# Changfei-Fu/RUMI-SLAM

Measured on AMD Instinct MI355X. Metric: frames/sec ORB extract+match, higher is better.
Workload: dtype u8; 1 GPU; ORB extract (640x480, 8-level pyramid, 1000 features/frame) + brute-force 256-bit Hamming match of consecutive frames (BASELINE.json configs[1]+[2]); scaling=n/a (one GPU), exchange=none

## Files before the change

rumi_slam_amd/csrc/orb_device.h:

```cpp
#pragma once
#include <hip/hip_runtime.h>

#include <cstdint>

#include "orb_geom.h"
#include "rumi_orb.h"

namespace rumi {

struct DevLevel {
    int w, h, pitch;
    long long off;
    int nCols, nRows, wCell, hCell;
    int cellBase, nCells;
    int maxBX, maxBY;
    int nfeat;
    float scale;
    float patchSize;
    int candCap;
    int coefX, coefXT, coefY, xmax;
    int xmaxFast;
    int rowTab;
};

struct DevParams {
    int nlevels, totalCells, maxCellCand, totalCand;
    int iniTh, minTh;
    long long arenaStride;
    int umax[16];
    DevLevel lv[kMaxLevels];
};

struct ImgSrc {
    const uint8_t *l0;
    long long l0FrameStride;
    int l0Pitch;
    uint8_t *pyr;
    uint8_t *blur;
};

struct RowTap { int32_t r0, r1; uint32_t bh0, bh1; };
struct PyrTile { int16_t x0[kMaxLevels], x1[kMaxLevels], y0[kMaxLevels], y1[kMaxLevels]; };
void launch_pyramid_tiles(const DevParams *dP, ImgSrc src, const int16_t *coef, const RowTap *rowTab, const PyrTile *tiles, int ntiles, int bufBytes,
                          int tabEntries, int nframes, hipStream_t st, int32_t *clearWord = nullptr, bool copyL0 = false);
void launch_resize(const DevParams *dP, const DevParams &hP, ImgSrc src, const int16_t *coef, const RowTap *rowTab, int level, int nframes,
                   hipStream_t st, int32_t *clearWord = nullptr);
void launch_fast(const DevParams *dP, const DevParams &hP, ImgSrc src, uint32_t *cellBuf, int32_t *cellCnt, int nframes,
                 hipStream_t st);
bool fast_blur_fusable(const DevParams &hP);
bool launch_fast_blur(const DevParams *dP, const DevParams &hP, ImgSrc src, uint32_t *cellBuf, int32_t *cellCnt, int nframes, int variant, hipStream_t st);
void launch_compact(const DevParams *dP, const DevParams &hP, const uint32_t *cellBuf, const int32_t *cellCnt,
                    uint32_t *cand, int32_t *levelStart, int32_t *errFlag, int nframes, hipStream_t st);
void launch_blur(const DevParams *dP, const DevParams &hP, ImgSrc src, int nframes, int variant, hipStream_t st);
void launch_orient_desc(const DevParams *dP, ImgSrc src, const uint32_t *selPacked, const uint32_t *selMeta,
                        const int32_t *selCount, int selCap, int maxSel, RumiKeyPoint *kpOut, long long kpStride, uint8_t *descOut,
                        long long descStride, int outCap, int nframes, hipStream_t st);

void launch_assemble_orient_desc(const DevParams *dP, ImgSrc src, const uint32_t *selLevel, const int32_t *selLevelCnt, int selLevelCap, int lap0, int lap1,
                                 int32_t *counts, long long countsStride, int32_t *errFlag, int32_t *errMirror, uint32_t *selPacked, uint32_t *selMeta,
                                 int32_t *selCount, int selCap, int maxSel, RumiKeyPoint *kpOut,
                                 long long kpStride, uint8_t *descOut, long long descStride, int outCap, int nframes, hipStream_t st);
void launch_octree(const DevParams *dP, const DevParams &hP, const uint32_t *cand, const int32_t *levelStart,
                   uint16_t *owner, uint32_t *selLevel, int32_t *selLevelCnt, int selLevelCap, int32_t *errFlag,
                   int nframes, size_t ldsBytes, hipStream_t st);
void launch_assemble(const DevParams *dP, const uint32_t *selLevel, const int32_t *selLevelCnt, int selLevelCap, int lap0,
                     int lap1, uint32_t *selPacked, uint32_t *selMeta, int32_t *selCount, int selCap, int32_t *counts, long long countsStride,
                     int32_t *errFlag, int nframes, hipStream_t st, int32_t *errMirror = nullptr);
size_t octree_lds_for(const DevParams &hP);

}
```

rumi_slam_amd/csrc/orb_host.hip:

```cpp
#include <hip/hip_runtime.h>

#include <cstdlib>

#include <algorithm>
#include <atomic>
#include <cstdio>
#include <cstring>
#include <functional>
#include <string>
#include <thread>
#include <vector>

#include "orb_device.h"
#include "orb_octree.h"
#include "rumi_common.h"

using namespace rumi;

namespace rumi {
thread_local std::string g_lastError;
void set_error(const char *fmt, const char *a, const char *b, int line) {
    char buf[512];
    snprintf(buf, sizeof buf, fmt, a, b, line);
    g_lastError = buf;
// ... 38 lines not shown
    RowTap *dRowTab = nullptr; int capRowTab = 0;
    PyrTile *dPyrTiles[2] = {nullptr, nullptr}; int nPyrTiles[2] = {0, 0}, pyrBuf[2] = {0, 0}, pyrTab[2] = {0, 0};
    uint8_t *dIn = nullptr;
    uint8_t *dL0 = nullptr;
    uint8_t *hIn = nullptr, *hOut1 = nullptr, *dOut1 = nullptr;
    size_t out1Bytes = 0;
    uint8_t *dhOut1 = nullptr;
    int32_t *dhErr = nullptr;
    bool zeroCopyOut = false;
    uint8_t *dhIn = nullptr;
    bool hostImagePending = false;
    uint8_t *dPyr = nullptr, *dBlur = nullptr;
    uint32_t *dCellBuf = nullptr;
    int32_t *dCellCnt = nullptr;
    uint32_t *dCand = nullptr;
    int32_t *dLevelStart = nullptr;
    uint32_t *dSelPacked = nullptr, *dSelMeta = nullptr;
    int32_t *dSelCount = nullptr;
    RumiKeyPoint *dKp = nullptr;
    uint8_t *dDesc = nullptr;
    int32_t *dCounts = nullptr;
    uint16_t *dOwner = nullptr;
    uint32_t *dSelLevel = nullptr;
    int32_t *dSelLevelCnt = nullptr;
    int32_t *dErr = nullptr;
    uint8_t *dHostIn = nullptr; size_t dHostInBytes = 0;
    static constexpr int kFeedSlots = 4, kFeedFrames = 64;
    uint8_t *hFeed[kFeedSlots] = {nullptr}; size_t hFeedBytes = 0;
    hipEvent_t evFeed[kFeedSlots] = {nullptr};
    hipStream_t copyStream = nullptr, copyStream2 = nullptr;
    std::function<int(int, hipStream_t)> feed;
    bool pending = false;
    hipStream_t pendingStream = nullptr;
    int selLevelCap = 0;
    size_t octLds = 0;
    int32_t *hErr = nullptr;
    std::vector<uint32_t> tapCand, tapSelPacked, tapSelMeta;
    std::vector<int32_t> tapLevelStart, tapSelCount;
    bool tapValid = false;
    ImgSrc lastSrc{};
    int lastFrames = 0, lastChunkBase = 0, lastChunkFrames = 0, lastChunkSlot = 0;
    RumiKeyPoint *lastKp = nullptr;
    long long lastKpStride = 0;
    int32_t *lastCounts = nullptr;
    int lastOutCap = 0;
    bool profiling = false;
    float stageMs[8] = {0};
    struct Mirror { uint8_t *host; const uint8_t *dev; long long row; } mirror[3] = {{nullptr, nullptr, 0}, {nullptr, nullptr, 0}, {nullptr, nullptr, 0}};
    hipEvent_t ev[8] = {nullptr};
    hipStream_t sideStream = nullptr;
    static constexpr int kMaxParts = 8;
    hipStream_t partStream[kMaxParts - 1] = {nullptr}, partSide[kMaxParts - 1] = {nullptr};
    bool residentQueue = false;
    int residentSlots = 4;
    int scratchFrames = 0, arenaFrames = 0;
    int rot = 0;
    hipEvent_t userReady = nullptr;
    bool lastResident = false;
    hipStream_t part0Stream = nullptr, part0Side = nullptr;
    hipEvent_t evPart0Join = nullptr, evSide0Fork = nullptr, evSide0Join = nullptr;
    hipEvent_t evPartFork = nullptr, evPartJoin[kMaxParts - 1] = {nullptr}, evSideFork[kMaxParts - 1] = {nullptr}, evSideJoin[kMaxParts - 1] = {nullptr};
    hipEvent_t evFork = nullptr, evJoin = nullptr, evB0 = nullptr, evB1 = nullptr;
};

static int set_geometry(RumiOrb *h, int w, int hgt) {
    if (h->gw == w && h->gh == hgt) return RUMI_OK;
    std::vector<LevelGeom> g;
    long long arena; int cells, cand, cellCand;
    if (!make_geometry(h->tab, w, hgt, g, &arena, &cells, &cand, &cellCand)) {
        g_lastError = "image too small for the FAST cell grid at some pyramid level, or cell larger than the LDS tile";
        return RUMI_E_INVALID;
    }
    if (arena > h->capArena || cells > h->capCells || cand > h->capCand || cellCand > h->capCellCand) {
        g_lastError = "image larger than the handle's max_width x max_height arenas";
        return RUMI_E_CAPACITY;
    }
    DevParams &P = h->hP;
    std::memset(&P, 0, sizeof P);
    P.nlevels = h->tab.nlevels; P.totalCells = cells; P.maxCellCand = h->capCellCand; P.totalCand = h->capCand;
    P.iniTh = std::min(std::max(h->cfg.ini_th_fast, 0), 255);
    P.minTh = std::min(std::max(h->cfg.min_th_fast, 0), 255);
    P.arenaStride = h->capArena;
    for (int i = 0; i < 16; i++) P.umax[i] = h->tab.umax[i];
    std::vector<int16_t> coef;
    std::vector<RowTap> rowTab;
    for (int l = 0; l < P.nlevels; l++) {
        DevLevel &D = P.lv[l];
        const LevelGeom &G = g[l];
        D.w = G.w; D.h = G.h; D.pitch = G.pitch; D.off = G.off;
        D.nCols = G.nCols; D.nRows = G.nRows; D.wCell = G.wCell; D.hCell = G.hCell;
        D.cellBase = G.cellBase; D.nCells = G.nCells; D.maxBX = G.maxBX; D.maxBY = G.maxBY;
        D.nfeat = G.nfeat; D.scale = G.scale;
        D.patchSize = (float)(int)(kPatchSize * G.scale);
        D.candCap = std::min(G.candCap, 65535);
        D.coefX = D.coefXT = D.coefY = 0; D.xmax = D.xmaxFast = G.w; D.rowTab = 0;
        if (l > 0) {
            std::vector<int16_t> ofs, taps;
            int dmax;
            make_resize_axis(g[l - 1].w, G.w, true, ofs, taps, &dmax);
            D.coefX = (int)coef.size(); D.xmax = dmax;
            D.xmaxFast = dmax == G.w ? G.w + 3 : dmax;
            for (int k = 0; k < 4; k++) { ofs.push_back(ofs[G.w - 1]); taps.push_back(taps[2 * G.w - 2]); taps.push_back(taps[2 * G.w - 1]); }
            coef.insert(coef.end(), ofs.begin(), ofs.end());
            D.coefXT = (int)coef.size();
            coef.insert(coef.end(), taps.begin(), taps.end());
            make_resize_axis(g[l - 1].h, G.h, false, ofs, taps, &dmax);
            D.coefY = (int)coef.size();
            coef.insert(coef.end(), ofs.begin(), ofs.end());
            coef.insert(coef.end(), taps.begin(), taps.end());
            D.rowTab = (int)rowTab.size();
            const int sh = g[l - 1].h;
            for (int oy = 0; oy < G.h; oy++) {
                const int sy = ofs[oy];
                const int sy0 = sy >= 0 ? (sy < sh ? sy : sh - 1) : 0, sy1r = sy + 1, sy1 = sy1r >= 0 ? (sy1r < sh ? sy1r : sh - 1) : 0;
                rowTab.push_back(RowTap{sy0, sy1, (uint32_t)taps[oy * 2] << 16, (uint32_t)taps[oy * 2 + 1] << 16});
            }
        }
    }
    if ((int)coef.size() > h->capCoef) { g_lastError = "resize table capacity"; return RUMI_E_CAPACITY; }
    HIP_TRY(hipMemcpy(h->dP, &P, sizeof P, hipMemcpyHostToDevice));
    if ((int)rowTab.size() > h->capRowTab) { g_lastError = "resize row table capacity"; return RUMI_E_CAPACITY; }
    if (!coef.empty()) HIP_TRY(hipMemcpy(h->dCoef, coef.data(), coef.size() * sizeof(int16_t), hipMemcpyHostToDevice));
    if (!rowTab.empty()) HIP_TRY(hipMemcpy(h->dRowTab, rowTab.data(), rowTab.size() * sizeof(RowTap), hipMemcpyHostToDevice));
    auto build_tiles = [&](int kPyrTX, int kPyrTY, int set) -> int {
        h->nPyrTiles[set] = 0; h->pyrBuf[set] = 0;
        if (P.nlevels < 2) return RUMI_OK;
        const int top = P.nlevels - 1;
        const int ntx = (P.lv[top].w + kPyrTX - 1) / kPyrTX, nty = (P.lv[top].h + kPyrTY - 1) / kPyrTY;
        std::vector<PyrTile> tiles((size_t)ntx * nty);
        int bufMax = 0, tabMax = 0, dimMax = 0, winRows = 0, winCols = 0;
        auto up4 = [](int x) { return (x + 3) & ~3; };
        for (int ty = 0; ty < nty; ty++)
            for (int tx = 0; tx < ntx; tx++) {
                PyrTile &T = tiles[(size_t)ty * ntx + tx];
                std::memset(&T, 0, sizeof T);
                int x0 = 0, x1 = 0, y0 = 0, y1 = 0, tab = 0;
                for (int l = top; l >= 0; l--) {
                    const DevLevel &D = P.lv[l];
                    int ox0 = (int)((long long)D.w * tx / ntx), ox1 = (int)((long long)D.w * (tx + 1) / ntx);
                    int oy0 = (int)((long long)D.h * ty / nty), oy1 = (int)((long long)D.h * (ty + 1) / nty);
                    if (l < top) {
                        const DevLevel &U = P.lv[l + 1];
                        const int16_t *xofs = coef.data() + U.coefX;
                        const int nx0 = xofs[x0], nx1 = std::min(D.w, (int)xofs[x1 - 1] + 2);
                        const int ny0 = rowTab[(size_t)U.rowTab + y0].r0, ny1 = rowTab[(size_t)U.rowTab + y1 - 1].r1 + 1;
                        if (l == 0) { ox0 = nx0; ox1 = nx1; oy0 = ny0; oy1 = ny1; }
                        else { ox0 = std::min(ox0, nx0); ox1 = std::max(ox1, nx1); oy0 = std::min(oy0, ny0); oy1 = std::max(oy1, ny1); }
                    }
                    if (l > 0) { x0 = ox0 & ~3; x1 = up4(ox1); } else { x0 = ox0 & ~3; x1 = ox1; }
                    y0 = oy0; y1 = oy1;
                    T.x0[l] = (int16_t)x0; T.x1[l] = (int16_t)x1; T.y0[l] = (int16_t)y0; T.y1[l] = (int16_t)y1;
                    bufMax = std::max(bufMax, up4(x1 - x0) * (y1 - y0));
                    if (l > 0) tab += (x1 - x0) + (y1 - y0);
                    if (l > 0) dimMax = std::max(dimMax, std::max(x1 - x0, y1 - y0));
                    if (l == 0) { winRows = std::max(winRows, y1 - y0); winCols = std::max(winCols, x1 - x0); }
                }
                tabMax = std::max(tabMax, tab);
            }
        bufMax = (bufMax + 15) & ~15;
        if (2 * bufMax + 8 * tabMax <= 60 * 1024 && tiles.size() <= 4096 && P.nlevels <= 8 && dimMax <= 256 && winRows <= 80 && winCols <= 256) {
            if (h->dPyrTiles[set]) { (void)hipFree(h->dPyrTiles[set]); h->dPyrTiles[set] = nullptr; }
            HIP_TRY(hipMalloc((void **)&h->dPyrTiles[set], tiles.size() * sizeof(PyrTile)));
            HIP_TRY(hipMemcpy(h->dPyrTiles[set], tiles.data(), tiles.size() * sizeof(PyrTile), hipMemcpyHostToDevice));
            h->nPyrTiles[set] = (int)tiles.size(); h->pyrBuf[set] = bufMax; h->pyrTab[set] = tabMax;
        }
        return RUMI_OK;
// ... 743 lines not shown
```

rumi_slam_amd/csrc/orb_kernels.hip:

```cpp
#include <hip/hip_runtime.h>

#include "orb_device.h"
#include "orb_math.h"

namespace rumi {

struct PatternF { float v[256 * 4]; };
constexpr PatternF make_pattern_f() {
    constexpr int8_t src[256 * 4] = {
#include "orb_pattern.inc"
    };
    PatternF p{};
    for (int i = 0; i < 256 * 4; i++) p.v[i] = (float)src[i];
    return p;
}
__constant__ PatternF c_patternF = make_pattern_f();

__device__ __forceinline__ unsigned xcd_swizzle(unsigned lin, unsigned total) {
    const unsigned q = total >> 3, r = total & 7, xcd = lin & 7;
    return (xcd < r ? xcd * (q + 1) : r * (q + 1) + (xcd - r) * q) + (lin >> 3);
}

struct __attribute__((packed)) U32 { uint32_t v; };
struct __attribute__((packed)) U64 { uint64_t v; };
// ... 803 lines not shown
            selA = (selA & ~(0xFFu << (8 * i))) | (a << (8 * i));
            selB = (selB & ~(0xFFu << (8 * i))) | (b << (8 * i));
        }
    }
    int ring[7][4];
#pragma unroll
    for (int k = 0; k < 7; k++)
#pragma unroll
        for (int i = 0; i < 4; i++) ring[k][i] = 0;
    const int yEnd = min(y0 + kBlurRows, h), rEnd = yEnd + 3;
    uint8_t *orow = out + (long long)(y0 - 6) * L.pitch + xa - L.pitch;
    const int haloOff = lane == 0 ? (firstBlock ? 0 : -4) : (lane == 63 && !edgeWave && bw == 256 ? 4 : 0);
    uint32_t Cn[7], Hn[7];
    auto fetch = [&](int r, uint32_t &C, uint32_t &H) {
        const int rc = min(r, rEnd - 1);
        const int rr = rc < 0 ? -rc : (rc >= h ? 2 * (h - 1) - rc : rc);
        const uint8_t *row = img + (long long)rr * pitch + xl;
        C = *reinterpret_cast<const uint32_t *>(row);
        H = 0;
        if (haloOff) H = *reinterpret_cast<const uint32_t *>(row + haloOff);
    };
#pragma unroll
    for (int j = 0; j < 7; j++) fetch(y0 - 3 + j, Cn[j], Hn[j]);
    uint32_t Cm[7], Hm[7];
    auto walk7 = [&](const uint32_t (&Cc)[7], const uint32_t (&Hc)[7], int r0) {
#pragma unroll
        for (int j = 0; j < 7; j++) {
            const int r = r0 + j;
            if (r >= rEnd) break;
            orow += L.pitch;
            uint32_t C = Cc[j];
            if (edgeWave) {
                const uint32_t c1 = __shfl_up(C, 1), c2 = __shfl_up(c1, 1);
                C = __builtin_amdgcn_perm(C, __builtin_amdgcn_perm(c1, c2, selA), selB);
            }
            uint32_t Lw = __shfl_up(C, 1), Rw = __shfl_down(C, 1);
            if (lane == 0) Lw = firstBlock ? __builtin_amdgcn_perm(C, C, 0x01020300u) : Hc[j];
            if (lane == 63 && !edgeWave && bw == 256) Rw = Hc[j];
            constexpr uint32_t tA = 18u | (34u << 8) | (kT2 << 16) | (kT3 << 24), tB = kT2 | (34u << 8) | (18u << 16);
            const uint32_t A0 = __builtin_amdgcn_alignbyte(C, Lw, 1), A1 = __builtin_amdgcn_alignbyte(C, Lw, 2), A2 = __builtin_amdgcn_alignbyte(C, Lw, 3);
            const uint32_t B0 = __builtin_amdgcn_alignbyte(Rw, C, 1), B1 = __builtin_amdgcn_alignbyte(Rw, C, 2), B2 = __builtin_amdgcn_alignbyte(Rw, C, 3);
            ring[j][0] = (int)__builtin_amdgcn_udot4(B0, tB, __builtin_amdgcn_udot4(A0, tA, 0u, false), false);
            ring[j][1] = (int)__builtin_amdgcn_udot4(B1, tB, __builtin_amdgcn_udot4(A1, tA, 0u, false), false);
            ring[j][2] = (int)__builtin_amdgcn_udot4(B2, tB, __builtin_amdgcn_udot4(A2, tA, 0u, false), false);
            ring[j][3] = (int)__builtin_amdgcn_udot4(Rw, tB, __builtin_amdgcn_udot4(C, tA, 0u, false), false);
            const int y = r - 3;
            if (y >= y0 && produce) {
                uint32_t o[4];
#pragma unroll
                for (int i = 0; i < 4; i++) {
                    uint32_t acc = mad_u24(kT3, (uint32_t)ring[(j + 4) % 7][i], 32768u);
                    acc = mad_u24(kT2, (uint32_t)(ring[(j + 3) % 7][i] + ring[(j + 5) % 7][i]), acc);
                    acc = mad_u24(34u, (uint32_t)(ring[(j + 2) % 7][i] + ring[(j + 6) % 7][i]), acc);
                    acc = mad_u24(18u, (uint32_t)(ring[(j + 1) % 7][i] + ring[j][i]), acc);
                    if (VARIANT) acc = min(acc, 0x00FFFFFFu);
                    o[i] = acc;
                }
                const uint32_t p01 = __builtin_amdgcn_perm(o[1], o[0], 0x0c0c0602u), p23 = __builtin_amdgcn_perm(o[3], o[2], 0x06020c0cu);
                *reinterpret_cast<uint32_t *>(orow) = p01 | p23;
            }
        }
    };
    for (int r0 = y0 - 3; r0 < rEnd; r0 += 7) {
#pragma unroll
        for (int j = 0; j < 7; j++) Cm[j] = Cn[j], Hm[j] = Hn[j];
        if (r0 + 7 < rEnd) {
#pragma unroll
            for (int j = 0; j < 7; j++) fetch(r0 + 7 + j, Cn[j], Hn[j]);
        }
        walk7(Cm, Hm, r0);
    }
}
template <int VARIANT, int kBlurRows>
__global__ __launch_bounds__(256) void k_blur(const DevParams *__restrict__ P, ImgSrc src, BlurGrid G) {
    blur_body<VARIANT, kBlurRows>(P, src, G, blockIdx.x, gridDim.x);
}
template <int TPC, int VARIANT, bool LEGACY>
__global__ __launch_bounds__(256) void k_fast_blur(const DevParams *__restrict__ P, ImgSrc src, FastLds F, uint32_t *__restrict__ cellBuf,
                                                   int32_t *__restrict__ cellCnt, BlurGrid G, unsigned gxFast) {
    if (blockIdx.x < gxFast) fast_cells_body<TPC, LEGACY>(P, src, F, cellBuf, cellCnt, blockIdx.x, gxFast);
    else blur_body<VARIANT, kBlurRowsSmall>(P, src, G, blockIdx.x - gxFast, gridDim.x - gxFast);
}

__device__ __forceinline__ int half_wave_sum(int v) {
    v += __builtin_amdgcn_update_dpp(0, v, 0x111, 0xF, 0xF, false);
    v += __builtin_amdgcn_update_dpp(0, v, 0x112, 0xF, 0xF, false);
    v += __builtin_amdgcn_update_dpp(0, v, 0x114, 0xF, 0xF, false);
    v += __builtin_amdgcn_update_dpp(0, v, 0x118, 0xF, 0xF, false);
    v += __builtin_amdgcn_update_dpp(0, v, 0x142, 0xA, 0xF, false);
    const int lo = __builtin_amdgcn_readlane(v, 31), hi = __builtin_amdgcn_readlane(v, 63);
    return (threadIdx.x & 32) ? hi : lo;
}
__device__ __forceinline__ int wave_sum(int v) {
#pragma unroll
    for (int o = 32; o > 0; o >>= 1) v += __shfl_xor(v, o);
    return v;
}

constexpr int kDiscP = 48, kPatchP = 48;
constexpr int kKpPerWg = 8;

struct AssembleArgs {
    const uint32_t *selLevel; const int32_t *selLevelCnt; int selLevelCap, lap0, lap1;
    int32_t *counts; long long countsStride; int32_t *errFlag, *errMirror;
    uint32_t *selPackedOut, *selMetaOut; int32_t *selCountOut;
};
template <int kKpGroups, bool kAssemble>
__global__ __launch_bounds__(256, 7) void k_orient_desc(const DevParams *__restrict__ P, ImgSrc src,
                                                     const uint32_t *__restrict__ selPacked,
                                                     const uint32_t *__restrict__ selMeta,
                                                     const int32_t *__restrict__ selCount, int selCap,
                                                     RumiKeyPoint *__restrict__ kpOut, long long kpStride, uint8_t *__restrict__ descOut,
                                                     long long descStride, int outCap, AssembleArgs A) {
    static_assert(kDiscP == kPatchP, "the disc and the patch share their rows");
    __shared__ __attribute__((aligned(16))) uint8_t sWin[kKpPerWg][37 * kPatchP];
    __shared__ __attribute__((aligned(16))) float sPat[256 * 4];
    __shared__ int4 sLv[kMaxLevels];
    __shared__ float2 sLvF[kMaxLevels];
    reinterpret_cast<float4 *>(sPat)[threadIdx.x] = reinterpret_cast<const float4 *>(c_patternF.v)[threadIdx.x];
    if (threadIdx.x < (unsigned)P->nlevels) {
        const DevLevel &Lv = P->lv[threadIdx.x];
        sLv[threadIdx.x] = threadIdx.x == 0 ? make_int4(0, src.l0Pitch, (int)Lv.off, Lv.pitch) : make_int4((int)Lv.off, Lv.pitch, (int)Lv.off, Lv.pitch);
        sLvF[threadIdx.x] = make_float2(Lv.scale, Lv.patchSize);
    }
    const int lane = threadIdx.x & 31, hw = threadIdx.x >> 5;
    const unsigned wg = xcd_swizzle(blockIdx.y * gridDim.x + blockIdx.x, gridDim.x * gridDim.y);
    const int kb = (wg % gridDim.x) * (kKpPerWg * kKpGroups) + hw, frame = wg / gridDim.x;
    int cnt;
    __shared__ uint32_t sOwnPk[kAssemble ? kKpPerWg * kKpGroups : 1], sOwnMt[kAssemble ? kKpPerWg * kKpGroups : 1];
    if constexpr (!kAssemble) {
        cnt = selCount[frame];
        __syncthreads();
    } else {
        __shared__ int sLvStart[kMaxLevels + 1], sRed[2], sOwnF[kKpPerWg * kKpGroups];
        const int nl = P->nlevels, tid = threadIdx.x;
        if (tid == 0) {
            int run = 0;
            for (int l = 0; l < nl; l++) { sLvStart[l] = run; run += A.selLevelCnt[(long long)frame * nl + l]; }
            sLvStart[nl] = run; sRed[0] = 0; sRed[1] = 0;
        }
        __syncthreads();
        const int total = sLvStart[nl], kbase = (wg % gridDim.x) * (kKpPerWg * kKpGroups);
        const bool first = wg % gridDim.x == 0, over = total > selCap;
        int32_t *counts = reinterpret_cast<int32_t *>(reinterpret_cast<uint8_t *>(A.counts) + frame * A.countsStride);
        if (over) {
            if (first && tid == 0) { A.selCountOut[frame] = 0; counts[0] = total; counts[1] = 0; const int old = atomicOr(A.errFlag, 8); if (A.errMirror) *A.errMirror = old | 8; }
            return;
        }
        cnt = total;
        auto key_at = [&](int k, int *levelOut) -> uint32_t {
            int level = 0;
            while (k >= sLvStart[level + 1]) level++;
            *levelOut = level;
            return A.selLevel[((long long)frame * nl + level) * A.selLevelCap + (k - sLvStart[level])];
        };
        auto lapped = [&](uint32_t pk, int level) -> bool {
            float x = (float)((int)(pk & 0xFFF) + kBorder);
            if (level != 0) x = x * P->lv[level].scale;
            return x >= (float)A.lap0 && x <= (float)A.lap1;
        };
        int before = 0, all = 0;
        for (int k = tid; k < total; k += 256) {
            int level;
            const uint32_t pk = key_at(k, &level);
            const int f = lapped(pk, level) ? 1 : 0;
            all += f; before += k < kbase ? f : 0;
        }
#pragma unroll
        for (int o = 32; o > 0; o >>= 1) { before += __shfl_xor(before, o); all += __shfl_xor(all, o); }
        if ((tid & 63) == 0) { atomicAdd(&sRed[0], before); atomicAdd(&sRed[1], all); }
        if (tid < kKpPerWg * kKpGroups) {
            const int k = kbase + tid;
            int level = 0;
            uint32_t pk = 0;
            int f = 0;
            if (k < total) { pk = key_at(k, &level); f = lapped(pk, level) ? 1 : 0; }
            sOwnPk[tid] = pk; sOwnMt[tid] = (uint32_t)level; sOwnF[tid] = f;
        }
        __syncthreads();
        if (tid == 0) {
            int b = sRed[0];
            for (int j = 0; j < kKpPerWg * kKpGroups; j++) {
                const int k = kbase + j;
                if (k >= total) break;
                const int f = sOwnF[j], slot = f ? (total - 1 - b) : (k - b);
                b += f;
                sOwnMt[j] |= (uint32_t)slot << 8;
            }
            if (first) {
                counts[0] = total; counts[1] = total - sRed[1];
// ... 38 lines not shown
        if (qRow) { S.q0 = ld16(br2); S.q1 = ld16(br2 + 16); S.q2 = ld8(br2 + 32); }
    };
    auto stage_disc = [&](bool live, const Staged &S) {
        if (!live || !dRow) return;
        uint8_t *dst = &sWin[hw][lane * kDiscP];
        *reinterpret_cast<uint4 *>(dst) = S.d0; *reinterpret_cast<uint4 *>(dst + 16) = S.d1; *reinterpret_cast<uint32_t *>(dst + 32) = S.d2;
    };
    auto stage_patch = [&](bool live, const Staged &S) {
        if (!live) return;
        {
            uint8_t *dst = &sWin[hw][lane * kPatchP];
            *reinterpret_cast<uint4 *>(dst) = S.p0; *reinterpret_cast<uint4 *>(dst + 16) = S.p1; *reinterpret_cast<uint2 *>(dst + 32) = S.p2;
        }
        if (qRow) {
            uint8_t *dst = &sWin[hw][(lane + 32) * kPatchP];
            *reinterpret_cast<uint4 *>(dst) = S.q0; *reinterpret_cast<uint4 *>(dst + 16) = S.q1; *reinterpret_cast<uint2 *>(dst + 32) = S.q2;
        }
    };
    auto orientation = [&](uint32_t pk) -> float {
        const int x = (int)(pk & 0xFFF) + kBorder;
        const int xd = (x - kHalfPatch) & ~3;
        const uint8_t *dc = &sWin[hw][kHalfPatch * kDiscP + (x - xd)];
        const int u = lane - kHalfPatch;
        const int vmaxU = lane < 31 ? P->umax[u < 0 ? -u : u] : -1;
        const int mid = dc[u];
        int colSum = vmaxU >= 0 ? mid : 0, m01 = 0;
#pragma unroll
        for (int v = 1; v <= kHalfPatch; v++) {
            const int lo = dc[-v * kDiscP + u], hi = dc[v * kDiscP + u];
            const bool in = v <= vmaxU;
            colSum += in ? lo + hi : 0;
            m01 += in ? v * (hi - lo) : 0;
        }
        int m10 = u * colSum;
        m10 = half_wave_sum(m10);
        m01 = half_wave_sum(m01);
        OD_STAMP(4);
        return fast_atan2_deg((float)m01, (float)m10);
    };
    auto describe = [&](uint32_t pk, uint32_t meta, float angle) {
        const int level = meta & 0xFF, slot = (int)(meta >> 8);
        const int x = (int)(pk & 0xFFF) + kBorder, y = (int)((pk >> 12) & 0xFFF) + kBorder, score = (int)(pk >> 24);
        const int xp = (x - 18) & ~3;
        const float factorPI = (float)(3.1415926535897932384626433832795 / 180.f);
        const float ang = angle * factorPI;
        const float a = cosf_glibc(ang), b = sinf_glibc(ang);
        const uint8_t *bc = &sWin[hw][18 * kPatchP + (x - xp)];
        uint32_t w = 0;
        OD_STAMP(5);
#pragma unroll
        for (int j = 0; j < 8; j++) {
            const float4 pt = reinterpret_cast<const float4 *>(sPat)[j * 32 + lane];
            const float x0 = pt.x, y0 = pt.y, x1 = pt.z, y1 = pt.w;
            const int r0 = cv_round_f(x0 * b + y0 * a), c0 = cv_round_f(x0 * a - y0 * b);
            const int r1 = cv_round_f(x1 * b + y1 * a), c1 = cv_round_f(x1 * a - y1 * b);
            const int t0 = bc[r0 * kPatchP + c0], t1 = bc[r1 * kPatchP + c1];
            const unsigned long long bal = __ballot(t0 < t1);
            const uint32_t lo = (uint32_t)bal, hi = (uint32_t)(bal >> 32);
            asm("s_nop 4\n\tv_writelane_b32 %0, %1, %3\n\tv_writelane_b32 %0, %2, %4" : "+v"(w) : "s"(lo), "s"(hi), "n"(j), "n"(32 + j));
        }
        OD_STAMP(6);
        if (slot < outCap) {
            if (lane < 8) reinterpret_cast<uint32_t *>(descOut + frame * descStride + (long long)slot * 32)[lane] = w;
            if (lane == 0) {
                RumiKeyPoint kp;
                kp.x = (float)x; kp.y = (float)y;
                const float2 lf = sLvF[level];
                if (level != 0) { kp.x = kp.x * lf.x; kp.y = kp.y * lf.x; }
                kp.size = lf.y;
                kp.angle = angle;
                kp.response = (float)score;
                kp.octave = level;
                kp.class_id = -1;
                reinterpret_cast<RumiKeyPoint *>(reinterpret_cast<uint8_t *>(kpOut) + frame * kpStride)[slot] = kp;
            }
        }
    };

    const uint32_t *selP = selPacked + (long long)frame * selCap, *selM = selMeta + (long long)frame * selCap;
    auto key_rec = [&](int k, uint32_t &pk, uint32_t &mt) {
        if constexpr (kAssemble) { const int j = k - (kb - hw); pk = sOwnPk[j]; mt = sOwnMt[j]; }
        else { pk = selP[k]; mt = selM[k]; }
    };
    bool liveC = kb < cnt, liveN = kb + kKpPerWg < cnt;
    uint32_t pkC = 0, mtC = 0, pkN = 0, mtN = 0;
    if (liveC) key_rec(kb, pkC, mtC);
    if (liveN && kKpGroups > 1) key_rec(kb + kKpPerWg, pkN, mtN);
    if (kKpGroups == 1) liveN = false;
    Staged S;
    fetch_disc(pkC, mtC, liveC, S);
    fetch_patch(pkC, mtC, liveC, S);
#pragma unroll
    for (int g = 0; g < kKpGroups; g++) {
        if (!__any(liveC)) break;
        OD_STAMP(0);
        stage_disc(liveC, S);
        OD_STAMP(1);
        const int k2 = kb + (g + 2) * kKpPerWg;
        const bool liveNN = g + 2 < kKpGroups && k2 < cnt;
        uint32_t pkNN = 0, mtNN = 0;
        if (liveNN) key_rec(k2, pkNN, mtNN);
        if (g + 1 < kKpGroups) fetch_disc(pkN, mtN, liveN, S);
        OD_STAMP(2);
        float angle = 0.f;
        if (liveC) angle = orientation(pkC);
        stage_patch(liveC, S);
        if (g + 1 < kKpGroups) fetch_patch(pkN, mtN, liveN, S);
        if (liveC) describe(pkC, mtC, angle);
        OD_STAMP(3);
        pkC = pkN; mtC = mtN; liveC = liveN;
        pkN = pkNN; mtN = mtNN; liveN = liveNN;
    }
#ifdef RUMI_OD_STAMP
    if (threadIdx.x == 0 && (blockIdx.x % 8) == 0 && blockIdx.y == 0) printf("od wg %d: loop-head %lld stage(wait loads) %lld issue-next %lld | IC_Angle %lld trig %lld rBRIEF %lld store %lld\n", (int)blockIdx.x, st[0], st[1], st[2], st[4], st[5], st[6], st[3]);
#endif
}

void launch_resize(const DevParams *dP, const DevParams &hP, ImgSrc src, const int16_t *coef, const RowTap *rowTab, int level, int nframes,
                   hipStream_t st, int32_t *clearWord) {
    static const int envRows = std::getenv("RUMI_RESIZE_ROWS") ? std::atoi(std::getenv("RUMI_RESIZE_ROWS")) : 0;
    const int rows = envRows ? envRows : (hP.lv[level].h >= 200 ? 8 : 4);
    dim3 g((hP.lv[level].w + 255) / 256, (hP.lv[level].h + 4 * rows - 1) / (4 * rows), nframes);
    if (rows == 8) hipLaunchKernelGGL(k_resize<8>, g, dim3(256), 0, st, dP, src, coef, rowTab, level, clearWord);
    else hipLaunchKernelGGL(k_resize<4>, g, dim3(256), 0, st, dP, src, coef, rowTab, level, clearWord);
}
void launch_pyramid_tiles(const DevParams *dP, ImgSrc src, const int16_t *coef, const RowTap *rowTab, const PyrTile *tiles, int ntiles, int bufBytes,
                          int tabEntries, int nframes, hipStream_t st, int32_t *clearWord, bool copyL0) {
    hipLaunchKernelGGL(k_pyramid_tiles, dim3(ntiles, nframes), dim3(256), (size_t)2 * bufBytes + (size_t)tabEntries * 8, st, dP, src, coef, rowTab, tiles, bufBytes, clearWord, copyL0 ? 1 : 0);
}
static FastLds fast_lds_of(const DevParams &hP) {
    int wMax = 0, hMax = 0;
    for (int l = 0; l < hP.nlevels; l++) { wMax = std::max(wMax, hP.lv[l].wCell); hMax = std::max(hMax, hP.lv[l].hCell); }
    FastLds F;
    F.tp = 4 * (((wMax + 3) >> 2) + 2);
    F.sp = F.tp;
    F.tileBytes = (hMax + 6) * F.tp;
    F.scBytes = ((hMax + 2) * F.sp + 15) & ~15;
    F.maxIters = (wMax * hMax + 63) / 64 + 1;
    F.tileBytes = (F.tileBytes + 15) & ~15;
    F.perWave = (F.tileBytes + F.scBytes + std::max(kRingCap * 2, F.maxIters * 8) + kScoredCap * 2 + 15) & ~15;
    return F;
}
static bool fast_legacy() {
    static const bool legacy = std::getenv("RUMI_FAST_LEGACY") && std::atoi(std::getenv("RUMI_FAST_LEGACY")) != 0;
    return legacy;
}
void launch_fast(const DevParams *dP, const DevParams &hP, ImgSrc src, uint32_t *cellBuf, int32_t *cellCnt, int nframes,
                 hipStream_t st) {
    const FastLds F = fast_lds_of(hP);
    const bool legacy = fast_legacy();
    const int wpg = 4;
    const dim3 grid((hP.totalCells + wpg - 1) / wpg, nframes);
    const size_t lds = (size_t)wpg * F.perWave;
#define RUMI_FAST_CASE(T)                                                                                                  \
    if (F.tp == T) {                                                                                                       \
        if (legacy) hipLaunchKernelGGL((k_fast_cells<T, true>), grid, dim3(64 * wpg), lds, st, dP, src, F, cellBuf, cellCnt);  \
        else hipLaunchKernelGGL((k_fast_cells<T, false>), grid, dim3(64 * wpg), lds, st, dP, src, F, cellBuf, cellCnt);        \
        return;                                                                                                            \
    }
    RUMI_FAST_CASE(48) RUMI_FAST_CASE(44) RUMI_FAST_CASE(52) RUMI_FAST_CASE(56)
#undef RUMI_FAST_CASE
    if (legacy) hipLaunchKernelGGL((k_fast_cells<0, true>), grid, dim3(64 * wpg), lds, st, dP, src, F, cellBuf, cellCnt);
    else hipLaunchKernelGGL((k_fast_cells<0, false>), grid, dim3(64 * wpg), lds, st, dP, src, F, cellBuf, cellCnt);
}
static int compactSlices(int nframes) {
    static const int env = std::getenv("RUMI_COMPACT_SLICES") ? std::atoi(std::getenv("RUMI_COMPACT_SLICES")) : 0;
    return env > 0 ? env : (nframes < 32 ? 32 : 8);
}
void launch_compact(const DevParams *dP, const DevParams &hP, const uint32_t *cellBuf, const int32_t *cellCnt,
                    uint32_t *cand, int32_t *levelStart, int32_t *errFlag, int nframes, hipStream_t st) {
    hipLaunchKernelGGL(k_compact, dim3(nframes, compactSlices(nframes)), dim3(kCompactThreads), (hP.totalCells + 1) * sizeof(int), st, dP, cellBuf, cellCnt,
                       cand, levelStart, errFlag);
}
static int blur_strip_width(int w) {
    for (int bw : {256, 240, 224, 208}) {
        const int r = w % bw;
        const bool partialInFirstLanes = r >= 1 && r <= 8;
        const bool lane63Halo = bw == 256 && (r >= 253 || r <= 3);
        if (!partialInFirstLanes && !lane63Halo) return bw;
    }
    return 192;
}
static BlurGrid blur_grid_of(const DevParams &hP, int rows, int *total) {
    BlurGrid G{};
    int run = 0;
    for (int l = 0; l < hP.nlevels; l++) {
        G.bw[l] = blur_strip_width(hP.lv[l].w);
        G.gx[l] = (hP.lv[l].w + G.bw[l] - 1) / G.bw[l];
        G.base[l] = run;
        run += G.gx[l] * ((hP.lv[l].h + 4 * rows - 1) / (4 * rows));
    }
    G.base[hP.nlevels] = run;
    *total = run;
    return G;
}
bool fast_blur_fusable(const DevParams &hP) { return fast_lds_of(hP).tp == 48; }
bool launch_fast_blur(const DevParams *dP, const DevParams &hP, ImgSrc src, uint32_t *cellBuf, int32_t *cellCnt, int nframes, int variant, hipStream_t st) {
    const FastLds F = fast_lds_of(hP);
    if (F.tp != 48) return false;
    int run = 0;
    const BlurGrid G = blur_grid_of(hP, kBlurRowsSmall, &run);
    const int wpg = 4;
    const unsigned gxFast = (unsigned)((hP.totalCells + wpg - 1) / wpg);
    const dim3 grid(gxFast + (unsigned)run, nframes);
    const size_t lds = (size_t)wpg * F.perWave;
    const bool legacy = fast_legacy();
    if (variant && legacy) hipLaunchKernelGGL((k_fast_blur<48, 1, true>), grid, dim3(256), lds, st, dP, src, F, cellBuf, cellCnt, G, gxFast);
    else if (variant) hipLaunchKernelGGL((k_fast_blur<48, 1, false>), grid, dim3(256), lds, st, dP, src, F, cellBuf, cellCnt, G, gxFast);
    else if (legacy) hipLaunchKernelGGL((k_fast_blur<48, 0, true>), grid, dim3(256), lds, st, dP, src, F, cellBuf, cellCnt, G, gxFast);
    else hipLaunchKernelGGL((k_fast_blur<48, 0, false>), grid, dim3(256), lds, st, dP, src, F, cellBuf, cellCnt, G, gxFast);
    return true;
}
void launch_blur(const DevParams *dP, const DevParams &hP, ImgSrc src, int nframes, int variant, hipStream_t st) {
    const bool small = nframes < 16;
    const int rows = small ? kBlurRowsSmall : kBlurRowsBatch;
    int run = 0;
    const BlurGrid G = blur_grid_of(hP, rows, &run);
    if (small) {
        if (variant) hipLaunchKernelGGL((k_blur<1, kBlurRowsSmall>), dim3(run, nframes), dim3(256), 0, st, dP, src, G);
        else hipLaunchKernelGGL((k_blur<0, kBlurRowsSmall>), dim3(run, nframes), dim3(256), 0, st, dP, src, G);
    } else {
        if (variant) hipLaunchKernelGGL((k_blur<1, kBlurRowsBatch>), dim3(run, nframes), dim3(256), 0, st, dP, src, G);
        else hipLaunchKernelGGL((k_blur<0, kBlurRowsBatch>), dim3(run, nframes), dim3(256), 0, st, dP, src, G);
    }
}
void launch_orient_desc(const DevParams *dP, ImgSrc src, const uint32_t *selPacked, const uint32_t *selMeta,
                        const int32_t *selCount, int selCap, int maxSel, RumiKeyPoint *kpOut, long long kpStride, uint8_t *descOut,
                        long long descStride, int outCap, int nframes, hipStream_t st) {
    if (maxSel <= 0) return;
    const int wg1 = (maxSel + kKpPerWg - 1) / kKpPerWg;
    const AssembleArgs none{};
    if ((long long)wg1 * nframes <= 2048)
        hipLaunchKernelGGL((k_orient_desc<1, false>), dim3(wg1, nframes), dim3(256), 0, st, dP, src, selPacked, selMeta, selCount, selCap, kpOut, kpStride, descOut,
                           descStride, outCap, none);
    else
        hipLaunchKernelGGL((k_orient_desc<2, false>), dim3((wg1 + 1) / 2, nframes), dim3(256), 0, st, dP, src, selPacked, selMeta, selCount, selCap, kpOut, kpStride,
                           descOut, descStride, outCap, none);
}
void launch_assemble_orient_desc(const DevParams *dP, ImgSrc src, const uint32_t *selLevel, const int32_t *selLevelCnt, int selLevelCap, int lap0, int lap1,
                                 int32_t *counts, long long countsStride, int32_t *errFlag, int32_t *errMirror, uint32_t *selPacked, uint32_t *selMeta,
                                 int32_t *selCount, int selCap, int maxSel, RumiKeyPoint *kpOut,
                                 long long kpStride, uint8_t *descOut, long long descStride, int outCap, int nframes, hipStream_t st) {
    if (maxSel <= 0) return;
    const int wg1 = (maxSel + kKpPerWg - 1) / kKpPerWg;
    const AssembleArgs A{selLevel, selLevelCnt, selLevelCap, lap0, lap1, counts, countsStride, errFlag, nframes == 1 ? errMirror : nullptr, selPacked, selMeta, selCount};
    hipLaunchKernelGGL((k_orient_desc<1, true>), dim3(wg1, nframes), dim3(256), 0, st, dP, src, (const uint32_t *)nullptr, (const uint32_t *)nullptr,
                       (const int32_t *)nullptr, selCap, kpOut, kpStride, descOut, descStride, outCap, A);
}

}
```

rumi_slam_amd/csrc/orb_math.h:

```cpp
#pragma once
#include <cfloat>
#include <cstdint>
#include <cstring>

#if defined(__HIPCC__)
#define RUMI_HD __host__ __device__ inline
#else
#define RUMI_HD inline
#endif

namespace rumi {

RUMI_HD int cv_round_f(float v) { return (int)__builtin_rintf(v); }

RUMI_HD float fast_atan2_deg(float y, float x) {
    const float kRad2Deg = (float)(180 / 3.1415926535897932384626433832795);
    const float p1 = 0.9997878412794807f * kRad2Deg;
    const float p3 = -0.3258083974640975f * kRad2Deg;
    const float p5 = 0.1555786518463281f * kRad2Deg;
    const float p7 = -0.04432655554792128f * kRad2Deg;
    const float ax = __builtin_fabsf(x), ay = __builtin_fabsf(y);
    float a, c, c2;
    if (ax >= ay) {
        c = ay / (ax + (float)DBL_EPSILON);
        c2 = c * c;
        a = (((p7 * c2 + p5) * c2 + p3) * c2 + p1) * c;
    } else {
        c = ax / (ay + (float)DBL_EPSILON);
        c2 = c * c;
        a = 90.f - (((p7 * c2 + p5) * c2 + p3) * c2 + p1) * c;
    }
    if (x < 0) a = 180.f - a;
    if (y < 0) a = 360.f - a;
    return a;
}

namespace sincosf_impl {
struct Tab { double c0, c1, c2, c3, c4, s1, s2, s3; };
RUMI_HD float poly(double x, double x2, bool negCos, int n) {
    const double sg = negCos ? -1.0 : 1.0;
    const double c0 = sg * 0x1p0, c1 = sg * -0x1.ffffffd0c621cp-2, c2c = sg * 0x1.55553e1068f19p-5,
                 c3 = sg * -0x1.6c087e89a359dp-10, c4 = sg * 0x1.99343027bf8c3p-16;
    const double s1c = -0x1.555545995a603p-3, s2c = 0x1.1107605230bc4p-7, s3c = -0x1.994eb3774cf24p-13;
    if ((n & 1) == 0) {
        double x3 = x * x2;
        double s1 = s2c + x2 * s3c;
        double x7 = x3 * x2;
        double s = x + x3 * s1c;
        return (float)(s + x7 * s1);
    } else {
        double x4 = x2 * x2;
        double cc2 = c3 + x2 * c4;
        double cc1 = c0 + x2 * c1;
        double x6 = x4 * x2;
        double c = cc1 + x4 * c2c;
        return (float)(c + x6 * cc2);
    }
}
RUMI_HD uint32_t top12(float f) {
    uint32_t u;
#if defined(__HIP_DEVICE_COMPILE__)
    u = __float_as_uint(f);
#else
    std::memcpy(&u, &f, 4);
#endif
    return (u >> 20) & 0x7ff;
}
RUMI_HD float eval(float y, int isCos) {
    double x = y;
    if (top12(y) < top12(0x1.921FB6p-1f)) {
        if (top12(y) < top12(0x1p-12f)) return isCos ? 1.0f : y;
        return poly(x, x * x, false, isCos);
    }
    const double r = x * 0x1.45F306DC9C883p+23;
    const int n = ((int32_t)r + 0x800000) >> 24;
    x = x - n * 0x1.921FB54442D18p0;
    const double s = ((n & 3) == 1 || (n & 3) == 2) ? -1.0 : 1.0;
    return poly(x * s, x * x, (n & 2) != 0, n ^ isCos);
}
}
RUMI_HD float sinf_glibc(float x) { return sincosf_impl::eval(x, 0); }
RUMI_HD float cosf_glibc(float x) { return sincosf_impl::eval(x, 1); }

}
```

Measured before the change: 288,500 frames/s.

## Restructure orient/descriptor kernel to batch keypoint groups and compute moments with byte dot ops

Adds a new default path in the orientation and descriptor kernel. It fetches the disc patches for all keypoint groups up front and computes IC_Angle moments with a precomputed disc byte mask using sad_u8 and udot4. It then computes all angles and sin/cos at once in spread lanes with a branchless atan2 and a combined sincos, and broadcasts them via readlane. The goal is to overlap loads and cut the per-keypoint serial dependency chain and divergent math, at the cost of more registers and code size. The old path stays available behind the RUMI_OD_LEGACY environment variable.

New measurement: 290,100 frames/s, median of 6. No clear change (+0.6%).

```diff
diff --git a/rumi_slam_amd/csrc/orb_device.h b/rumi_slam_amd/csrc/orb_device.h
--- a/rumi_slam_amd/csrc/orb_device.h
+++ b/rumi_slam_amd/csrc/orb_device.h
@@ -29,6 +29,7 @@
     long long arenaStride;
     int umax[16];
     DevLevel lv[kMaxLevels];
+    uint32_t discMask[32][8];
 };
 
 struct ImgSrc {
diff --git a/rumi_slam_amd/csrc/orb_host.hip b/rumi_slam_amd/csrc/orb_host.hip
--- a/rumi_slam_amd/csrc/orb_host.hip
+++ b/rumi_slam_amd/csrc/orb_host.hip
@@ -144,6 +144,11 @@
     P.minTh = std::min(std::max(h->cfg.min_th_fast, 0), 255);
     P.arenaStride = h->capArena;
     for (int i = 0; i < 16; i++) P.umax[i] = h->tab.umax[i];
+    for (int r = 0; r < 2 * kHalfPatch + 1; r++)
+        for (int b = 0; b < 2 * kHalfPatch + 1; b++) {
+            const int v = std::abs(r - kHalfPatch), u = std::abs(b - kHalfPatch);
+            if (u <= P.umax[v]) P.discMask[r][b >> 2] |= 0xFFu << (8 * (b & 3));
+        }
     std::vector<int16_t> coef;
     std::vector<RowTap> rowTab;
     for (int l = 0; l < P.nlevels; l++) {
diff --git a/rumi_slam_amd/csrc/orb_kernels.hip b/rumi_slam_amd/csrc/orb_kernels.hip
--- a/rumi_slam_amd/csrc/orb_kernels.hip
+++ b/rumi_slam_amd/csrc/orb_kernels.hip
@@ -909,13 +909,17 @@
     else blur_body<VARIANT, kBlurRowsSmall>(P, src, G, blockIdx.x - gxFast, gridDim.x - gxFast);
 }
 
-__device__ __forceinline__ int half_wave_sum(int v) {
+__device__ __forceinline__ void half_wave_sums(int v, int &lo, int &hi) {
     v += __builtin_amdgcn_update_dpp(0, v, 0x111, 0xF, 0xF, false);
     v += __builtin_amdgcn_update_dpp(0, v, 0x112, 0xF, 0xF, false);
     v += __builtin_amdgcn_update_dpp(0, v, 0x114, 0xF, 0xF, false);
     v += __builtin_amdgcn_update_dpp(0, v, 0x118, 0xF, 0xF, false);
     v += __builtin_amdgcn_update_dpp(0, v, 0x142, 0xA, 0xF, false);
-    const int lo = __builtin_amdgcn_readlane(v, 31), hi = __builtin_amdgcn_readlane(v, 63);
+    lo = __builtin_amdgcn_readlane(v, 31); hi = __builtin_amdgcn_readlane(v, 63);
+}
+__device__ __forceinline__ int half_wave_sum(int v) {
+    int lo, hi;
+    half_wave_sums(v, lo, hi);
     return (threadIdx.x & 32) ? hi : lo;
 }
 __device__ __forceinline__ int wave_sum(int v) {
@@ -932,7 +936,7 @@
     int32_t *counts; long long countsStride; int32_t *errFlag, *errMirror;
     uint32_t *selPackedOut, *selMetaOut; int32_t *selCountOut;
 };
-template <int kKpGroups, bool kAssemble>
+template <int kKpGroups, bool kAssemble, bool kLegacy>
 __global__ __launch_bounds__(256, 7) void k_orient_desc(const DevParams *__restrict__ P, ImgSrc src,
                                                      const uint32_t *__restrict__ selPacked,
                                                      const uint32_t *__restrict__ selMeta,
@@ -1137,6 +1141,7 @@
         if constexpr (kAssemble) { const int j = k - (kb - hw); pk = sOwnPk[j]; mt = sOwnMt[j]; }
         else { pk = selP[k]; mt = selM[k]; }
     };
+    if constexpr (kLegacy) {
     bool liveC = kb < cnt, liveN = kb + kKpPerWg < cnt;
     uint32_t pkC = 0, mtC = 0, pkN = 0, mtN = 0;
     if (liveC) key_rec(kb, pkC, mtC);
@@ -1166,8 +1171,124 @@
         pkC = pkN; mtC = mtN; liveC = liveN;
         pkN = pkNN; mtN = mtNN; liveN = liveNN;
     }
+    } else {
+    const uint4 mkA = ld16(reinterpret_cast<const uint8_t *>(&P->discMask[lane][0])), mkB = ld16(reinterpret_cast<const uint8_t *>(&P->discMask[lane][4]));
+    auto moments = [&](uint32_t pk, const Staged &S, int &m10, int &m01) {
+        const uint32_t o = (uint32_t)((int)(pk & 0xFFF) + kBorder - kHalfPatch) & 3u;
+        const uint32_t w[9] = {S.d0.x, S.d0.y, S.d0.z, S.d0.w, S.d1.x, S.d1.y, S.d1.z, S.d1.w, S.d2};
+        const uint32_t mk[8] = {mkA.x, mkA.y, mkA.z, mkA.w, mkB.x, mkB.y, mkB.z, mkB.w};
+        uint32_t sum = 0, dot = 0;
+#pragma unroll
+        for (int i = 0; i < 8; i++) {
+            const uint32_t q = __builtin_amdgcn_alignbyte(w[i + 1], w[i], o) & mk[i];
+            sum = __builtin_amdgcn_sad_u8(q, 0u, sum);
+            dot = __builtin_amdgcn_udot4(q, 0x03020100u + 0x04040404u * (uint32_t)i, dot, false);
+        }
+        m10 = __mul24(-kHalfPatch, (int)sum) + (int)dot;
+        m01 = __mul24(lane - kHalfPatch, (int)sum);
+    };
+    auto describe_rows = [&](uint32_t pk, uint32_t meta, float angle, float a, float b) {
+        const int level = meta & 0xFF, slot = (int)(meta >> 8);
+        const int x = (int)(pk & 0xFFF) + kBorder, y = (int)((pk >> 12) & 0xFFF) + kBorder, score = (int)(pk >> 24);
+        const int xp = (x - 18) & ~3;
+        const uint32_t base = (uint32_t)(hw * 37 * kPatchP + 18 * kPatchP + (x - xp)) - (uint32_t)kPatchP * (uint32_t)kRoundBias
+                              - (0x4B000000u + (uint32_t)kRoundBias);
+        const uint8_t *win = &sWin[0][0];
+        typedef float f2 __attribute__((ext_vector_type(2)));
+        const f2 ba = {b, a}, aNb = {a, -b}, magic = {kRoundMagic, kRoundMagic};
+        auto offset = [&](float px, float py) -> uint32_t {
+            const f2 t = (f2{px, px} * ba + f2{py, py} * aNb) + magic;
+            return mad_u24(__float_as_uint(t.x), kPatchP, __float_as_uint(t.y)) + base;
+        };
+        uint32_t w = 0;
+#pragma unroll
+        for (int j = 0; j < 8; j++) {
+            const float4 pt = reinterpret_cast<const float4 *>(sPat)[j * 32 + lane];
+            const int t0 = win[offset(pt.x, pt.y)], t1 = win[offset(pt.z, pt.w)];
+            const unsigned long long bal = __ballot(t0 < t1);
+            const uint32_t lo = (uint32_t)bal, hi = (uint32_t)(bal >> 32);
+            asm("s_nop 4\n\tv_writelane_b32 %0, %1, %3\n\tv_writelane_b32 %0, %2, %4" : "+v"(w) : "s"(lo), "s"(hi), "n"(j), "n"(32 + j));
+        }
+        OD_STAMP(6);
+        if (slot < outCap) {
+            if (lane < 8) reinterpret_cast<uint32_t *>(descOut + frame * descStride + (long long)slot * 32)[lane] = w;
+            if (lane == 0) {
+                RumiKeyPoint kp;
+                kp.x = (float)x; kp.y = (float)y;
+                const float2 lf = sLvF[level];
+                if (level != 0) { kp.x = kp.x * lf.x; kp.y = kp.y * lf.x; }
+                kp.size = lf.y;
+                kp.angle = angle;
+                kp.response = (float)score;
+                kp.octave = level;
+                kp.class_id = -1;
+                reinterpret_cast<RumiKeyPoint *>(reinterpret_cast<uint8_t *>(kpOut) + frame * kpStride)[slot] = kp;
+            }
+        }
+    };
+    bool live[kKpGroups];
+    uint32_t pks[kKpGroups], mts[kKpGroups];
+    Staged S[kKpGroups];
+#pragma unroll
+    for (int g = 0; g < kKpGroups; g++) {
+        live[g] = kb + g * kKpPerWg < cnt;
+        pks[g] = 0; mts[g] = 0;
+        S[g].d0 = S[g].d1 = make_uint4(0, 0, 0, 0); S[g].d2 = 0;
+        if (live[g]) key_rec(kb + g * kKpPerWg, pks[g], mts[g]);
+    }
+    if (!__any(live[0])) return;
+#pragma unroll
+    for (int g = 0; g < kKpGroups; g++) fetch_disc(pks[g], mts[g], live[g], S[g]);
+    fetch_patch(pks[0], mts[0], live[0], S[0]);
+    OD_STAMP(0);
+    int s10[kKpGroups][2], s01[kKpGroups][2];
+#pragma unroll
+    for (int g = 0; g < kKpGroups; g++) {
+        int m10, m01;
+        moments(pks[g], S[g], m10, m01);
+        half_wave_sums(m10, s10[g][0], s10[g][1]);
+        half_wave_sums(m01, s01[g][0], s01[g][1]);
+    }
+    OD_STAMP(4);
+    const int wl = threadIdx.x & 63;
+    int my10 = s10[0][0], my01 = s01[0][0];
+#pragma unroll
+    for (int i = 1; i < 2 * kKpGroups; i++) {
+        my10 = wl == i ? s10[i >> 1][i & 1] : my10;
+        my01 = wl == i ? s01[i >> 1][i & 1] : my01;
+    }
+    const float factorPI = (float)(3.1415926535897932384626433832795 / 180.f);
+    const float myAngle = fast_atan2_deg_sel((float)my01, (float)my10);
+    float mySin, myCos;
+    sincosf_glibc(myAngle * factorPI, &mySin, &myCos);
+    const bool upper = (threadIdx.x & 32) != 0;
+    float angK[kKpGroups], aK[kKpGroups], bK[kKpGroups];
+#pragma unroll
+    for (int g = 0; g < kKpGroups; g++) {
+        const int l0 = 2 * g, l1 = 2 * g + 1;
+        const int an0 = __builtin_amdgcn_readlane(__float_as_int(myAngle), l0), an1 = __builtin_amdgcn_readlane(__float_as_int(myAngle), l1);
+        const int c0 = __builtin_amdgcn_readlane(__float_as_int(myCos), l0), c1 = __builtin_amdgcn_readlane(__float_as_int(myCos), l1);
+        const int s0 = __builtin_amdgcn_readlane(__float_as_int(mySin), l0), s1 = __builtin_amdgcn_readlane(__float_as_int(mySin), l1);
+        angK[g] = __int_as_float(upper ? an1 : an0);
+        aK[g] = __int_as_float(upper ? c1 : c0);
+        bK[g] = __int_as_float(upper ? s1 : s0);
+    }
+    OD_STAMP(5);
+#pragma unroll
+    for (int g = 0; g < kKpGroups; g++) {
+        if (g > 0 && !__any(live[g])) break;
+        stage_patch(live[g], S[g]);
+        if (g + 1 < kKpGroups) fetch_patch(pks[g + 1], mts[g + 1], live[g + 1], S[g + 1]);
+        OD_STAMP(1);
+        if (live[g]) describe_rows(pks[g], mts[g], angK[g], aK[g], bK[g]);
+        OD_STAMP(3);
+    }
+    }
 #ifdef RUMI_OD_STAMP
-    if (threadIdx.x == 0 && (blockIdx.x % 8) == 0 && blockIdx.y == 0) printf("od wg %d: loop-head %lld stage(wait loads) %lld issue-next %lld | IC_Angle %lld trig %lld rBRIEF %lld store %lld\n", (int)blockIdx.x, st[0], st[1], st[2], st[4], st[5], st[6], st[3]);
+    if (threadIdx.x == 0 && (blockIdx.x % 8) == 0 && blockIdx.y == 0) {
+        if (kLegacy) printf("od wg %d: loop-head %lld stage(wait loads) %lld issue-next %lld | IC_Angle %lld trig %lld rBRIEF %lld store %lld\n", (int)blockIdx.x, st[0], st[1], st[2], st[4], st[5], st[6], st[3]);
+        else printf("od-reg wg %d: issue loads %lld | IC_Angle (wait discs) %lld trig %lld | stage patch (wait) %lld rBRIEF %lld store %lld\n", (int)blockIdx.x, st[0], st[4], st[5], st[1], st[6], st[3]);
+    }
 #endif
 }
 
@@ -1279,18 +1400,30 @@
         else hipLaunchKernelGGL((k_blur<0, kBlurRowsBatch>), dim3(run, nframes), dim3(256), 0, st, dP, src, G);
     }
 }
+static bool od_legacy() {
+    static const bool legacy = std::getenv("RUMI_OD_LEGACY") && std::atoi(std::getenv("RUMI_OD_LEGACY")) != 0;
+    return legacy;
+}
 void launch_orient_desc(const DevParams *dP, ImgSrc src, const uint32_t *selPacked, const uint32_t *selMeta,
                         const int32_t *selCount, int selCap, int maxSel, RumiKeyPoint *kpOut, long long kpStride, uint8_t *descOut,
                         long long descStride, int outCap, int nframes, hipStream_t st) {
     if (maxSel <= 0) return;
     const int wg1 = (maxSel + kKpPerWg - 1) / kKpPerWg;
     const AssembleArgs none{};
-    if ((long long)wg1 * nframes <= 2048)
-        hipLaunchKernelGGL((k_orient_desc<1, false>), dim3(wg1, nframes), dim3(256), 0, st, dP, src, selPacked, selMeta, selCount, selCap, kpOut, kpStride, descOut,
-                           descStride, outCap, none);
-    else
-        hipLaunchKernelGGL((k_orient_desc<2, false>), dim3((wg1 + 1) / 2, nframes), dim3(256), 0, st, dP, src, selPacked, selMeta, selCount, selCap, kpOut, kpStride,
-                           descOut, descStride, outCap, none);
+    const bool legacy = od_legacy();
+    if ((long long)wg1 * nframes <= 2048) {
+        const dim3 grid(wg1, nframes);
+        if (legacy) hipLaunchKernelGGL((k_orient_desc<1, false, true>), grid, dim3(256), 0, st, dP, src, selPacked, selMeta, selCount, selCap, kpOut, kpStride,
+                                       descOut, descStride, outCap, none);
+        else hipLaunchKernelGGL((k_orient_desc<1, false, false>), grid, dim3(256), 0, st, dP, src, selPacked, selMeta, selCount, selCap, kpOut, kpStride,
+                                descOut, descStride, outCap, none);
+    } else {
+        const dim3 grid((wg1 + 1) / 2, nframes);
+        if (legacy) hipLaunchKernelGGL((k_orient_desc<2, false, true>), grid, dim3(256), 0, st, dP, src, selPacked, selMeta, selCount, selCap, kpOut, kpStride,
+                                       descOut, descStride, outCap, none);
+        else hipLaunchKernelGGL((k_orient_desc<2, false, false>), grid, dim3(256), 0, st, dP, src, selPacked, selMeta, selCount, selCap, kpOut, kpStride,
+                                descOut, descStride, outCap, none);
+    }
 }
 void launch_assemble_orient_desc(const DevParams *dP, ImgSrc src, const uint32_t *selLevel, const int32_t *selLevelCnt, int selLevelCap, int lap0, int lap1,
                                  int32_t *counts, long long countsStride, int32_t *errFlag, int32_t *errMirror, uint32_t *selPacked, uint32_t *selMeta,
@@ -1299,8 +1432,12 @@
     if (maxSel <= 0) return;
     const int wg1 = (maxSel + kKpPerWg - 1) / kKpPerWg;
     const AssembleArgs A{selLevel, selLevelCnt, selLevelCap, lap0, lap1, counts, countsStride, errFlag, nframes == 1 ? errMirror : nullptr, selPacked, selMeta, selCount};
-    hipLaunchKernelGGL((k_orient_desc<1, true>), dim3(wg1, nframes), dim3(256), 0, st, dP, src, (const uint32_t *)nullptr, (const uint32_t *)nullptr,
-                       (const int32_t *)nullptr, selCap, kpOut, kpStride, descOut, descStride, outCap, A);
-}
-
-}
+    if (od_legacy())
+        hipLaunchKernelGGL((k_orient_desc<1, true, true>), dim3(wg1, nframes), dim3(256), 0, st, dP, src, (const uint32_t *)nullptr, (const uint32_t *)nullptr,
+                           (const int32_t *)nullptr, selCap, kpOut, kpStride, descOut, descStride, outCap, A);
+    else
+        hipLaunchKernelGGL((k_orient_desc<1, true, false>), dim3(wg1, nframes), dim3(256), 0, st, dP, src, (const uint32_t *)nullptr, (const uint32_t *)nullptr,
+                           (const int32_t *)nullptr, selCap, kpOut, kpStride, descOut, descStride, outCap, A);
+}
+
+}
diff --git a/rumi_slam_amd/csrc/orb_math.h b/rumi_slam_amd/csrc/orb_math.h
--- a/rumi_slam_amd/csrc/orb_math.h
+++ b/rumi_slam_amd/csrc/orb_math.h
@@ -30,6 +30,23 @@
         c2 = c * c;
         a = 90.f - (((p7 * c2 + p5) * c2 + p3) * c2 + p1) * c;
     }
+    if (x < 0) a = 180.f - a;
+    if (y < 0) a = 360.f - a;
+    return a;
+}
+
+RUMI_HD float fast_atan2_deg_sel(float y, float x) {
+    const float kRad2Deg = (float)(180 / 3.1415926535897932384626433832795);
+    const float p1 = 0.9997878412794807f * kRad2Deg;
+    const float p3 = -0.3258083974640975f * kRad2Deg;
+    const float p5 = 0.1555786518463281f * kRad2Deg;
+    const float p7 = -0.04432655554792128f * kRad2Deg;
+    const float ax = __builtin_fabsf(x), ay = __builtin_fabsf(y);
+    const bool xMajor = ax >= ay;
+    const float c = (xMajor ? ay : ax) / ((xMajor ? ax : ay) + (float)DBL_EPSILON);
+    const float c2 = c * c;
+    const float p = (((p7 * c2 + p5) * c2 + p3) * c2 + p1) * c;
+    float a = xMajor ? p : 90.f - p;
     if (x < 0) a = 180.f - a;
     if (y < 0) a = 360.f - a;
     return a;
@@ -82,4 +99,35 @@
 RUMI_HD float sinf_glibc(float x) { return sincosf_impl::eval(x, 0); }
 RUMI_HD float cosf_glibc(float x) { return sincosf_impl::eval(x, 1); }
 
+RUMI_HD void sincosf_glibc(float y, float *sinOut, float *cosOut) {
+    using namespace sincosf_impl;
+    double x = y;
+    int n = 0;
+    if (top12(y) >= top12(0x1.921FB6p-1f)) {
+        const double r = x * 0x1.45F306DC9C883p+23;
+        n = ((int32_t)r + 0x800000) >> 24;
+        x = x - n * 0x1.921FB54442D18p0;
+    }
+    const double s = ((n & 3) == 1 || (n & 3) == 2) ? -1.0 : 1.0;
+    const double xs = x * s, x2 = x * x;
+    const bool neg = (n & 2) != 0;
+    const float ps = poly(xs, x2, neg, 0), pc = poly(xs, x2, neg, 1);
+    const bool tiny = top12(y) < top12(0x1p-12f);
+    *sinOut = tiny ? y : ((n & 1) ? pc : ps);
+    *cosOut = tiny ? 1.0f : ((n & 1) ? ps : pc);
 }
+
+constexpr float kRoundMagic = 0x1.8p23f;
+constexpr int kRoundBias = 1 << 22;
+RUMI_HD uint32_t round_magic_bits(float v) {
+    const float t = v + kRoundMagic;
+    uint32_t u;
+#if defined(__HIP_DEVICE_COMPILE__)
+    u = __float_as_uint(t);
+#else
+    std::memcpy(&u, &t, 4);
+#endif
+    return u;
+}
+
+}
```
